# veeresht/CommPy

Measured on AMD Instinct MI355X. Metric: decoded info-bits/s at fixed Eb/N0 (Viterbi K=7 r=1/2, 1024b); BER match, higher is better.
Workload: dtype f64

## Files before the change

### commpy_amd/csrc/viterbi_cw.hip

```cpp
#include "cpx_internal.h"
#include "cpx_math.h"
#include "viterbi_cw_asm.h"
#ifndef CPX_GEN_GB
#define CPX_GEN_GB 2
#endif

#include <atomic>
#include <cstdlib>
#include <cstring>
#include <mutex>
#include <type_traits>

using namespace cpx;

namespace {

template <int LGS, unsigned G0, unsigned G1>
struct SrCode {
    static constexpr int S = 1 << LGS;
    static constexpr int parity(unsigned v) { return __builtin_popcount(v) & 1; }
    static constexpr int code(int s, int j) {
        const unsigned p = (unsigned)(((s << 1) & (S - 1)) | j), b = (unsigned)(s >> (LGS - 1));
        const unsigned reg = (b << LGS) | p;
        return (parity(reg & G0) << 1) | parity(reg & G1);
// ... 54 lines not shown
        m0 = (double)(ri ^ 0ll);
        m1 = (double)(ri ^ 1ll);
    } else if (type == CPX_VIT_SOFT) {
        double nll0 = fast_log<false>(exp(r) + 1.0);
        m0 = nll0;
        m1 = nll0 - r;
    } else {
        double d0 = r - (-1.0), d1 = r - 1.0;
        m0 = d0 * d0;
        m1 = d1 * d1;
    }
}

__device__ __forceinline__ double clip500(double r) {
    double c;
    asm("v_max_f64 %0, %1, %2\n\tv_min_f64 %0, %0, %3" : "=&v"(c) : "v"(r), "s"(-500.0), "s"(500.0));
    return c;
}
__device__ __forceinline__ void soft_metrics_lean(double r, double &m0, double &m1) {
    const double nll0 = fast_log<false, false, true>(exp_pm500(r) + 1.0);
    m0 = nll0;
    m1 = nll0 - r;
}

template <int LGS>
__device__ __forceinline__ unsigned tb_hop(unsigned long long w, unsigned st) {
    const unsigned hi = (unsigned)((w << (st & ((1u << LGS) - 1u))) >> 32);
    return __builtin_amdgcn_alignbit(st, hi, 31);
}

struct NoHook {
    template <int P> __device__ __forceinline__ void at() const {}
};

template <int LGS, unsigned G0, unsigned G1, int TYPE, int R, bool LEAN = false, class Hook = NoHook>
__device__ __forceinline__ void cw_step(double (&pm)[1 << LGS], double r0, double r1, unsigned long long &word, int &best,
                                        const Hook &hook = Hook(), unsigned char *bml = nullptr, const unsigned *gidx = nullptr) {
    constexpr int type = TYPE;
    using C = SrCode<LGS, G0, G1>;
    constexpr bool GEN = G0 == 0 && G1 == 0;
    constexpr int S = 1 << LGS, H = S / 2;
    double m00, m01, m10, m11;
    if constexpr (LEAN && TYPE == CPX_VIT_SOFT) {
        r0 = clip500(r0);
        r1 = clip500(r1);
        soft_metrics_lean(r0, m00, m01);
        soft_metrics_lean(r1, m10, m11);
    } else {
        if (type == CPX_VIT_SOFT) {
            r0 = fmin(fmax(r0, -500.0), 500.0);
            r1 = fmin(fmax(r1, -500.0), 500.0);
        }
        bit_metrics_cw(type, r0, m00, m01);
        bit_metrics_cw(type, r1, m10, m11);
    }
    double bmv[4];
    if constexpr (LEAN) {
        bmv[0] = m00 + m10; bmv[1] = m00 + m11;
        bmv[2] = m01 + m10; bmv[3] = m01 + m11;
    } else {
        bmv[0] = (0.0 + m00) + m10; bmv[1] = (0.0 + m00) + m11;
        bmv[2] = (0.0 + m01) + m10; bmv[3] = (0.0 + m01) + m11;
    }
    unsigned da = 0, db = 0;
    hook.template at<0>();
    auto butterfly = [&](int j, double m_a0, double m_a1, double m_b0, double m_b1) {
        const int x = rotl<LGS>(2 * j, R), y = rotl<LGS>(2 * j + 1, R);
        const double a = pm[x], b = pm[y];
        const double a0 = a + m_a0, a1 = b + m_a1;
        const double b0 = a + m_b0, b1 = b + m_b1;
        if (TYPE == CPX_VIT_UNQUANTIZED) {
            pm[x] = acs_select(da, a0, a1);
            pm[y] = acs_select(db, b0, b1);
        } else {
            pm[x] = acs_min(da, a0, a1);
            pm[y] = acs_min(db, b0, b1);
        }
    };
    if constexpr (GEN) {
        typedef double cpx_d4 __attribute__((ext_vector_type(4)));
        const cpx_d4 tab = {bmv[0], bmv[1], bmv[2], bmv[3]}, rtab = {bmv[3], bmv[2], bmv[1], bmv[0]};
        asm volatile("s_set_gpr_idx_on 0, 1" ::: "memory", "m0");
        auto acs_pair = [&](int j, double a0, double a1, double b0, double b1) {
            const int x = rotl<LGS>(2 * j, R), y = rotl<LGS>(2 * j + 1, R);
            if (TYPE == CPX_VIT_UNQUANTIZED) {
                pm[x] = acs_select(da, a0, a1);
                pm[y] = acs_select(db, b0, b1);
            } else {
                pm[x] = acs_min(da, a0, a1);
                pm[y] = acs_min(db, b0, b1);
            }
        };
        if constexpr (H >= 4 && TYPE != CPX_VIT_UNQUANTIZED) {
#pragma unroll
            for (int j = 0; j < H; j += 2) {
                if (j == H / 2) hook.template at<1>();
                const int x0 = rotl<LGS>(2 * j, R), y0 = rotl<LGS>(2 * j + 1, R), x1 = rotl<LGS>(2 * j + 2, R), y1 = rotl<LGS>(2 * j + 3, R);
                const double a = pm[x0], b = pm[y0], c = pm[x1], d = pm[y1];
                double a0, a1, b0, b1, c0, c1, d0, d1;
                asm volatile("s_set_gpr_idx_idx %[i0]\n\t"
                             "v_add_f64 %[a0], v[248:249], %[a]\n\t"
                             "v_add_f64 %[b1], v[248:249], %[b]\n\t"
                             "v_add_f64 %[a1], v[240:241], %[b]\n\t"
                             "v_add_f64 %[b0], v[240:241], %[a]\n\t"
                             "s_set_gpr_idx_idx %[i1]\n\t"
                             "v_add_f64 %[c0], v[248:249], %[c]\n\t"
                             "v_add_f64 %[d1], v[248:249], %[d]\n\t"
                             "v_add_f64 %[c1], v[240:241], %[d]\n\t"
                             "v_add_f64 %[d0], v[240:241], %[c]\n\t"
                             "s_set_gpr_idx_idx 0\n\t"
                             "v_cmp_lt_f64 vcc, %[a1], %[a0]\n\tv_addc_co_u32 %[da], vcc, %[da], %[da], vcc\n\tv_min_f64 %[a0], %[a0], %[a1]\n\t"
                             "v_cmp_lt_f64 vcc, %[b1], %[b0]\n\tv_addc_co_u32 %[db], vcc, %[db], %[db], vcc\n\tv_min_f64 %[b0], %[b0], %[b1]\n\t"
                             "v_cmp_lt_f64 vcc, %[c1], %[c0]\n\tv_addc_co_u32 %[da], vcc, %[da], %[da], vcc\n\tv_min_f64 %[c0], %[c0], %[c1]\n\t"
                             "v_cmp_lt_f64 vcc, %[d1], %[d0]\n\tv_addc_co_u32 %[db], vcc, %[db], %[db], vcc\n\tv_min_f64 %[d0], %[d0], %[d1]"
                             : [a0] "=&v"(a0), [a1] "=&v"(a1), [b0] "=&v"(b0), [b1] "=&v"(b1), [c0] "=&v"(c0), [c1] "=&v"(c1),
                               [d0] "=&v"(d0), [d1] "=&v"(d1), [da] "+v"(da), [db] "+v"(db)
                             : [i0] "s"(gidx[j]), [i1] "s"(gidx[j + 1]), [a] "v"(a), [b] "v"(b), [c] "v"(c), [d] "v"(d),
                               "{v[248:255]}"(tab), "{v[240:247]}"(rtab)
                             : "vcc", "m0");
                pm[x0] = a0; pm[y0] = b0;
                pm[x1] = c0; pm[y1] = d0;
            }
        } else {
#pragma unroll
            for (int j = 0; j < H; j++) {
                if (j == H / 2) hook.template at<1>();
                const double a = pm[rotl<LGS>(2 * j, R)], b = pm[rotl<LGS>(2 * j + 1, R)];
                double a0, a1, b0, b1;
                asm volatile("s_set_gpr_idx_idx %[ic]\n\t"
                             "v_add_f64 %[a0], v[248:249], %[a]\n\t"
                             "v_add_f64 %[b1], v[248:249], %[b]\n\t"
                             "v_add_f64 %[a1], v[240:241], %[b]\n\t"
                             "v_add_f64 %[b0], v[240:241], %[a]\n\t"
                             "s_set_gpr_idx_idx 0"
                             : [a0] "=&v"(a0), [a1] "=&v"(a1), [b0] "=&v"(b0), [b1] "=&v"(b1)
                             : [ic] "s"(gidx[j]), [a] "v"(a), [b] "v"(b), "{v[248:255]}"(tab), "{v[240:247]}"(rtab)
                             : "m0");
                acs_pair(j, a0, a1, b0, b1);
            }
        }
        asm volatile("s_set_gpr_idx_off" ::: "memory", "m0");
    } else {
#pragma unroll
        for (int j = 0; j < H; j++) {
            if (j == H / 2) hook.template at<1>();
            butterfly(j, bmv[C::code(j, 0)], bmv[C::code(j, 1)], bmv[C::code(j + H, 0)], bmv[C::code(j + H, 1)]);
        }
    }
    hook.template at<2>();
    int bst = 0;
    constexpr bool ARGMIN32 = LEAN && S == 64 && TYPE == CPX_VIT_SOFT && !GEN;
    unsigned long long tie = ~0ull;
    if constexpr (ARGMIN32) {
        unsigned h0, h1, h2, h3;
#define CPX_H4(a) "v"(__double2hiint(pm[a])), "v"(__double2hiint(pm[(a) + 1])), "v"(__double2hiint(pm[(a) + 2])), "v"(__double2hiint(pm[(a) + 3]))
        asm(CPX_HMIN_BLOCK0 : "=&v"(h0), "=&v"(h1), "=&v"(h2), "=&v"(h3) : CPX_H4(0), CPX_H4(4), CPX_H4(8), CPX_H4(12), CPX_H4(16));
        asm(CPX_HMIN_BLOCK1 : "+v"(h0), "+v"(h1), "+v"(h2), "+v"(h3) : CPX_H4(20), CPX_H4(24), CPX_H4(28), CPX_H4(32), CPX_H4(36), CPX_H4(40));
        asm(CPX_HMIN_BLOCK2 : "+v"(h0), "+v"(h1), "+v"(h2), "+v"(h3) : CPX_H4(44), CPX_H4(48), CPX_H4(52), CPX_H4(56), CPX_H4(60));
#undef CPX_H4
        hook.template at<3>();
        unsigned ha, hb, tmp;
#define CPX_P1(a) "v"(__double2hiint(pm[rotl<LGS>((a), R + 1)])), "v"(__double2hiint(pm[rotl<LGS>((a) + 32, R + 1)]))
#define CPX_P4(a) CPX_P1(a), CPX_P1((a) + 1), CPX_P1((a) + 2), CPX_P1((a) + 3)
        asm(CPX_HIT_BLOCK0 : "=&v"(ha), "=&v"(hb) : "v"(h0), CPX_P4(0), CPX_P4(4), CPX_P4(8) : "vcc");
        asm(CPX_HIT_BLOCK1 : "+v"(ha), "+v"(hb) : "v"(h0), CPX_P4(12), CPX_P4(16), CPX_P4(20) : "vcc");
        asm(CPX_HIT_BLOCK2 : "+v"(ha), "+v"(hb), "=&v"(bst), "=&v"(tmp), "=&s"(tie) : "v"(h0), CPX_P4(24), CPX_P4(28) : "vcc");
#undef CPX_P4
#undef CPX_P1
    }
    if (__builtin_expect(tie != 0, !ARGMIN32)) {
        double m0 = pm[0], m1 = pm[1 % S], m2 = pm[2 % S], m3 = pm[3 % S];
        if constexpr (S == 64) {
#define CPX_V4(a) "v"(pm[a]), "v"(pm[(a) + 1]), "v"(pm[(a) + 2]), "v"(pm[(a) + 3])
            asm(CPX_MIN_BLOCK24 : "+v"(m0), "+v"(m1), "+v"(m2), "+v"(m3)
                : CPX_V4(4), CPX_V4(8), CPX_V4(12), CPX_V4(16), CPX_V4(20), CPX_V4(24));
            asm(CPX_MIN_BLOCK24 : "+v"(m0), "+v"(m1), "+v"(m2), "+v"(m3)
                : CPX_V4(28), CPX_V4(32), CPX_V4(36), CPX_V4(40), CPX_V4(44), CPX_V4(48));
            asm(CPX_MIN_BLOCK12 : "+v"(m0), "+v"(m1), "+v"(m2), "+v"(m3) : CPX_V4(52), CPX_V4(56), CPX_V4(60));
#undef CPX_V4
        } else {
#pragma unroll
            for (int s = 4; s < S; s += 4) {
                m0 = vmin(m0, pm[s]); m1 = vmin(m1, pm[s + 1]); m2 = vmin(m2, pm[s + 2]); m3 = vmin(m3, pm[s + 3]);
            }
        }
        const double mn = vmin(vmin(m0, m1), vmin(m2, m3));
        if constexpr (!ARGMIN32) hook.template at<3>();
        if constexpr (S == 64) {
            unsigned long long k0, k1, k2, k3;
#define CPX_S4(a) "v"(pm[rotl<LGS>((a), R + 1)]), "v"(pm[rotl<LGS>((a) - 1, R + 1)]), "v"(pm[rotl<LGS>((a) - 2, R + 1)]), "v"(pm[rotl<LGS>((a) - 3, R + 1)])
            asm(CPX_SCAN_BLOCK0 : "+v"(bst), "=&s"(k0), "=&s"(k1), "=&s"(k2), "=&s"(k3)
                : "v"(mn), CPX_S4(63), CPX_S4(59), CPX_S4(55), CPX_S4(51), CPX_S4(47), CPX_S4(43));
            asm(CPX_SCAN_BLOCK1 : "+v"(bst), "=&s"(k0), "=&s"(k1), "=&s"(k2), "=&s"(k3)
                : "v"(mn), CPX_S4(39), CPX_S4(35), CPX_S4(31), CPX_S4(27), CPX_S4(23), CPX_S4(19));
            asm(CPX_SCAN_BLOCK2 : "+v"(bst), "=&s"(k0), "=&s"(k1), "=&s"(k2), "=&s"(k3)
                : "v"(mn), CPX_S4(15), CPX_S4(11), CPX_S4(7), CPX_S4(3));
#undef CPX_S4
        } else if constexpr (S % 4 == 0) {
#pragma unroll
            for (int s = S - 4; s >= 0; s -= 4) {
                unsigned long long k0, k1, k2, k3;
                asm("v_cmp_eq_f64 %1, %5, %9\n\tv_cmp_eq_f64 %2, %6, %9\n\tv_cmp_eq_f64 %3, %7, %9\n\tv_cmp_eq_f64 %4, %8, %9\n\t"
                    "v_cndmask_b32 %0, %0, %10, %1\n\tv_cndmask_b32 %0, %0, %11, %2\n\tv_cndmask_b32 %0, %0, %12, %3\n\t"
                    "v_cndmask_b32 %0, %0, %13, %4"
                    : "+v"(bst), "=&s"(k0), "=&s"(k1), "=&s"(k2), "=&s"(k3)
                    : "v"(pm[rotl<LGS>(s + 3, R + 1)]), "v"(pm[rotl<LGS>(s + 2, R + 1)]), "v"(pm[rotl<LGS>(s + 1, R + 1)]),
                      "v"(pm[rotl<LGS>(s, R + 1)]), "v"(mn), "n"(s + 3), "n"(s + 2), "n"(s + 1), "n"(s));
            }
        } else {
#pragma unroll
            for (int s = S - 1; s >= 0; s--) bst = (pm[rotl<LGS>(s, R + 1)] == mn) ? s : bst;
        }
    }
    word = ((unsigned long long)da << (64 - H)) | ((unsigned long long)db << (64 - S));
    best = bst;
}

__device__ __forceinline__ float acs_min_f32(unsigned &acc, float x, float y) {
    float r;
    asm("v_cmp_lt_f32 vcc, %3, %2\n\tv_addc_co_u32 %1, vcc, %1, %1, vcc\n\tv_min_f32 %0, %2, %3"
        : "=&v"(r), "+v"(acc) : "v"(x), "v"(y) : "vcc");
    return r;
}
__device__ __forceinline__ float vmin3_f32(float a, float b, float c) {
    float r;
    asm("v_min3_f32 %0, %1, %2, %3" : "=v"(r) : "v"(a), "v"(b), "v"(c));
    return r;
}
__device__ __forceinline__ void bit_metrics_f32(int type, double r, float &m0, float &m1) {
    if (type == CPX_VIT_HARD) {
        const long long ri = (long long)r;
        m0 = (float)(ri ^ 0ll);
        m1 = (float)(ri ^ 1ll);
    } else if (type == CPX_VIT_SOFT) {
        m0 = 0.0f;
        m1 = -(float)r;
    } else {
        const float x = (float)r, d0 = x + 1.0f, d1 = x - 1.0f;
        m0 = d0 * d0;
        m1 = d1 * d1;
    }
}

template <int LGS, unsigned G0, unsigned G1, int TYPE, int R, bool LEAN = false, class Hook = NoHook>
__device__ __forceinline__ void cw_step(float (&pm)[1 << LGS], double r0, double r1, unsigned long long &word, int &best,
                                        const Hook &hook = Hook(), unsigned char * = nullptr, const unsigned * = nullptr) {
    using C = SrCode<LGS, G0, G1>;
    constexpr int S = 1 << LGS, H = S / 2;
    if (TYPE == CPX_VIT_SOFT) {
        r0 = fmin(fmax(r0, -500.0), 500.0);
        r1 = fmin(fmax(r1, -500.0), 500.0);
    }
    float m00, m01, m10, m11;
    bit_metrics_f32(TYPE, r0, m00, m01);
    bit_metrics_f32(TYPE, r1, m10, m11);
    float bmv[4];
    bmv[0] = (0.0f + m00) + m10; bmv[1] = (0.0f + m00) + m11;
    bmv[2] = (0.0f + m01) + m10; bmv[3] = (0.0f + m01) + m11;
    unsigned da = 0, db = 0;
    hook.template at<0>();
#pragma unroll
    for (int j = 0; j < H; j++) {
        if (j == H / 2) hook.template at<1>();
        const int x = rotl<LGS>(2 * j, R), y = rotl<LGS>(2 * j + 1, R);
        const float a = pm[x], b = pm[y];
        const float a0 = a + bmv[C::code(j, 0)], a1 = b + bmv[C::code(j, 1)];
        const float b0 = a + bmv[C::code(j + H, 0)], b1 = b + bmv[C::code(j + H, 1)];
        pm[x] = acs_min_f32(da, a0, a1);
        pm[y] = acs_min_f32(db, b0, b1);
    }
    hook.template at<2>();
    float mn;
    if constexpr (S >= 8 && S % 8 == 0) {
        float m0 = pm[0], m1 = pm[1], m2 = pm[2], m3 = pm[3];
#pragma unroll
        for (int s = 4; s + 8 <= S; s += 8) {
            m0 = vmin3_f32(m0, pm[s], pm[s + 1]); m1 = vmin3_f32(m1, pm[s + 2], pm[s + 3]);
            m2 = vmin3_f32(m2, pm[s + 4], pm[s + 5]); m3 = vmin3_f32(m3, pm[s + 6], pm[s + 7]);
        }
        m0 = vmin3_f32(m0, pm[S - 4], pm[S - 3]);
        m1 = vmin3_f32(m1, pm[S - 2], pm[S - 1]);
        mn = fminf(vmin3_f32(m0, m1, m2), m3);
    } else {
        mn = pm[0];
#pragma unroll
        for (int s = 1; s < S; s++) mn = fminf(mn, pm[s]);
    }
    hook.template at<3>();
    int bst = 0;
    if constexpr (S % 4 == 0) {
#pragma unroll
        for (int s = S - 4; s >= 0; s -= 4) {
            unsigned long long k0, k1, k2, k3;
            asm("v_cmp_eq_f32 %1, %5, %9\n\tv_cmp_eq_f32 %2, %6, %9\n\tv_cmp_eq_f32 %3, %7, %9\n\tv_cmp_eq_f32 %4, %8, %9\n\t"
                "v_cndmask_b32 %0, %0, %10, %1\n\tv_cndmask_b32 %0, %0, %11, %2\n\tv_cndmask_b32 %0, %0, %12, %3\n\t"
                "v_cndmask_b32 %0, %0, %13, %4"
                : "+v"(bst), "=&s"(k0), "=&s"(k1), "=&s"(k2), "=&s"(k3)
                : "v"(pm[rotl<LGS>(s + 3, R + 1)]), "v"(pm[rotl<LGS>(s + 2, R + 1)]), "v"(pm[rotl<LGS>(s + 1, R + 1)]),
                  "v"(pm[rotl<LGS>(s, R + 1)]), "v"(mn), "n"(s + 3), "n"(s + 2), "n"(s + 1), "n"(s));
        }
    } else {
#pragma unroll
        for (int s = S - 1; s >= 0; s--) bst = (pm[rotl<LGS>(s, R + 1)] == mn) ? s : bst;
    }
    word = ((unsigned long long)da << (64 - H)) | ((unsigned long long)db << (64 - S));
    best = bst;
}

constexpr int ACS_WAVES = 4;

template <int LGS, unsigned G0, unsigned G1, int TYPE>
__global__ __launch_bounds__(64 * ACS_WAVES) void viterbi_cw_acs_kernel(CwParams p) {
    constexpr int S = 1 << LGS;
    const int lane = threadIdx.x & 63;
    const int64_t grp = (int64_t)blockIdx.x * ACS_WAVES + (threadIdx.x >> 6);
    const int64_t cw = grp * 64 + lane;
    if (grp * 64 >= p.B) return;
    const bool valid = cw < p.B;
    const double *x = p.coded + (valid ? cw : 0) * p.len;
    unsigned long long *dec = p.dec + grp * p.Tp * 64 + lane;
    unsigned char *best = p.best + grp * p.Tp * 64 + lane;
// ... 620 lines not shown
```

### commpy_amd/csrc/viterbi_cw_asm.h

```cpp
#pragma once
#define CPX_MIN_BLOCK24 "v_min_f64 %0, %0, %4\n\tv_min_f64 %1, %1, %5\n\tv_min_f64 %2, %2, %6\n\tv_min_f64 %3, %3, %7\n\tv_min_f64 %0, %0, %8\n\tv_min_f64 %1, %1, %9\n\tv_min_f64 %2, %2, %10\n\tv_min_f64 %3, %3, %11\n\tv_min_f64 %0, %0, %12\n\tv_min_f64 %1, %1, %13\n\tv_min_f64 %2, %2, %14\n\tv_min_f64 %3, %3, %15\n\tv_min_f64 %0, %0, %16\n\tv_min_f64 %1, %1, %17\n\tv_min_f64 %2, %2, %18\n\tv_min_f64 %3, %3, %19\n\tv_min_f64 %0, %0, %20\n\tv_min_f64 %1, %1, %21\n\tv_min_f64 %2, %2, %22\n\tv_min_f64 %3, %3, %23\n\tv_min_f64 %0, %0, %24\n\tv_min_f64 %1, %1, %25\n\tv_min_f64 %2, %2, %26\n\tv_min_f64 %3, %3, %27"
#define CPX_MIN_BLOCK12 "v_min_f64 %0, %0, %4\n\tv_min_f64 %1, %1, %5\n\tv_min_f64 %2, %2, %6\n\tv_min_f64 %3, %3, %7\n\tv_min_f64 %0, %0, %8\n\tv_min_f64 %1, %1, %9\n\tv_min_f64 %2, %2, %10\n\tv_min_f64 %3, %3, %11\n\tv_min_f64 %0, %0, %12\n\tv_min_f64 %1, %1, %13\n\tv_min_f64 %2, %2, %14\n\tv_min_f64 %3, %3, %15"
#define CPX_SCAN_BLOCK0 "v_cmp_eq_f64 %1, %6, %5\n\tv_cmp_eq_f64 %2, %7, %5\n\tv_cmp_eq_f64 %3, %8, %5\n\tv_cmp_eq_f64 %4, %9, %5\n\tv_cndmask_b32 %0, %0, 63, %1\n\tv_cndmask_b32 %0, %0, 62, %2\n\tv_cndmask_b32 %0, %0, 61, %3\n\tv_cndmask_b32 %0, %0, 60, %4\n\tv_cmp_eq_f64 %1, %10, %5\n\tv_cmp_eq_f64 %2, %11, %5\n\tv_cmp_eq_f64 %3, %12, %5\n\tv_cmp_eq_f64 %4, %13, %5\n\tv_cndmask_b32 %0, %0, 59, %1\n\tv_cndmask_b32 %0, %0, 58, %2\n\tv_cndmask_b32 %0, %0, 57, %3\n\tv_cndmask_b32 %0, %0, 56, %4\n\tv_cmp_eq_f64 %1, %14, %5\n\tv_cmp_eq_f64 %2, %15, %5\n\tv_cmp_eq_f64 %3, %16, %5\n\tv_cmp_eq_f64 %4, %17, %5\n\tv_cndmask_b32 %0, %0, 55, %1\n\tv_cndmask_b32 %0, %0, 54, %2\n\tv_cndmask_b32 %0, %0, 53, %3\n\tv_cndmask_b32 %0, %0, 52, %4\n\tv_cmp_eq_f64 %1, %18, %5\n\tv_cmp_eq_f64 %2, %19, %5\n\tv_cmp_eq_f64 %3, %20, %5\n\tv_cmp_eq_f64 %4, %21, %5\n\tv_cndmask_b32 %0, %0, 51, %1\n\tv_cndmask_b32 %0, %0, 50, %2\n\tv_cndmask_b32 %0, %0, 49, %3\n\tv_cndmask_b32 %0, %0, 48, %4\n\tv_cmp_eq_f64 %1, %22, %5\n\tv_cmp_eq_f64 %2, %23, %5\n\tv_cmp_eq_f64 %3, %24, %5\n\tv_cmp_eq_f64 %4, %25, %5\n\tv_cndmask_b32 %0, %0, 47, %1\n\tv_cndmask_b32 %0, %0, 46, %2\n\tv_cndmask_b32 %0, %0, 45, %3\n\tv_cndmask_b32 %0, %0, 44, %4\n\tv_cmp_eq_f64 %1, %26, %5\n\tv_cmp_eq_f64 %2, %27, %5\n\tv_cmp_eq_f64 %3, %28, %5\n\tv_cmp_eq_f64 %4, %29, %5\n\tv_cndmask_b32 %0, %0, 43, %1\n\tv_cndmask_b32 %0, %0, 42, %2\n\tv_cndmask_b32 %0, %0, 41, %3\n\tv_cndmask_b32 %0, %0, 40, %4"
#define CPX_SCAN_BLOCK1 "v_cmp_eq_f64 %1, %6, %5\n\tv_cmp_eq_f64 %2, %7, %5\n\tv_cmp_eq_f64 %3, %8, %5\n\tv_cmp_eq_f64 %4, %9, %5\n\tv_cndmask_b32 %0, %0, 39, %1\n\tv_cndmask_b32 %0, %0, 38, %2\n\tv_cndmask_b32 %0, %0, 37, %3\n\tv_cndmask_b32 %0, %0, 36, %4\n\tv_cmp_eq_f64 %1, %10, %5\n\tv_cmp_eq_f64 %2, %11, %5\n\tv_cmp_eq_f64 %3, %12, %5\n\tv_cmp_eq_f64 %4, %13, %5\n\tv_cndmask_b32 %0, %0, 35, %1\n\tv_cndmask_b32 %0, %0, 34, %2\n\tv_cndmask_b32 %0, %0, 33, %3\n\tv_cndmask_b32 %0, %0, 32, %4\n\tv_cmp_eq_f64 %1, %14, %5\n\tv_cmp_eq_f64 %2, %15, %5\n\tv_cmp_eq_f64 %3, %16, %5\n\tv_cmp_eq_f64 %4, %17, %5\n\tv_cndmask_b32 %0, %0, 31, %1\n\tv_cndmask_b32 %0, %0, 30, %2\n\tv_cndmask_b32 %0, %0, 29, %3\n\tv_cndmask_b32 %0, %0, 28, %4\n\tv_cmp_eq_f64 %1, %18, %5\n\tv_cmp_eq_f64 %2, %19, %5\n\tv_cmp_eq_f64 %3, %20, %5\n\tv_cmp_eq_f64 %4, %21, %5\n\tv_cndmask_b32 %0, %0, 27, %1\n\tv_cndmask_b32 %0, %0, 26, %2\n\tv_cndmask_b32 %0, %0, 25, %3\n\tv_cndmask_b32 %0, %0, 24, %4\n\tv_cmp_eq_f64 %1, %22, %5\n\tv_cmp_eq_f64 %2, %23, %5\n\tv_cmp_eq_f64 %3, %24, %5\n\tv_cmp_eq_f64 %4, %25, %5\n\tv_cndmask_b32 %0, %0, 23, %1\n\tv_cndmask_b32 %0, %0, 22, %2\n\tv_cndmask_b32 %0, %0, 21, %3\n\tv_cndmask_b32 %0, %0, 20, %4\n\tv_cmp_eq_f64 %1, %26, %5\n\tv_cmp_eq_f64 %2, %27, %5\n\tv_cmp_eq_f64 %3, %28, %5\n\tv_cmp_eq_f64 %4, %29, %5\n\tv_cndmask_b32 %0, %0, 19, %1\n\tv_cndmask_b32 %0, %0, 18, %2\n\tv_cndmask_b32 %0, %0, 17, %3\n\tv_cndmask_b32 %0, %0, 16, %4"
#define CPX_SCAN_BLOCK2 "v_cmp_eq_f64 %1, %6, %5\n\tv_cmp_eq_f64 %2, %7, %5\n\tv_cmp_eq_f64 %3, %8, %5\n\tv_cmp_eq_f64 %4, %9, %5\n\tv_cndmask_b32 %0, %0, 15, %1\n\tv_cndmask_b32 %0, %0, 14, %2\n\tv_cndmask_b32 %0, %0, 13, %3\n\tv_cndmask_b32 %0, %0, 12, %4\n\tv_cmp_eq_f64 %1, %10, %5\n\tv_cmp_eq_f64 %2, %11, %5\n\tv_cmp_eq_f64 %3, %12, %5\n\tv_cmp_eq_f64 %4, %13, %5\n\tv_cndmask_b32 %0, %0, 11, %1\n\tv_cndmask_b32 %0, %0, 10, %2\n\tv_cndmask_b32 %0, %0, 9, %3\n\tv_cndmask_b32 %0, %0, 8, %4\n\tv_cmp_eq_f64 %1, %14, %5\n\tv_cmp_eq_f64 %2, %15, %5\n\tv_cmp_eq_f64 %3, %16, %5\n\tv_cmp_eq_f64 %4, %17, %5\n\tv_cndmask_b32 %0, %0, 7, %1\n\tv_cndmask_b32 %0, %0, 6, %2\n\tv_cndmask_b32 %0, %0, 5, %3\n\tv_cndmask_b32 %0, %0, 4, %4\n\tv_cmp_eq_f64 %1, %18, %5\n\tv_cmp_eq_f64 %2, %19, %5\n\tv_cmp_eq_f64 %3, %20, %5\n\tv_cmp_eq_f64 %4, %21, %5\n\tv_cndmask_b32 %0, %0, 3, %1\n\tv_cndmask_b32 %0, %0, 2, %2\n\tv_cndmask_b32 %0, %0, 1, %3\n\tv_cndmask_b32 %0, %0, 0, %4"
#define CPX_HMIN_BLOCK0 "v_min3_u32 %0, %4, %8, %12\n\tv_min3_u32 %1, %5, %9, %13\n\tv_min3_u32 %2, %6, %10, %14\n\tv_min3_u32 %3, %7, %11, %15\n\tv_min3_u32 %0, %0, %16, %20\n\tv_min3_u32 %1, %1, %17, %21\n\tv_min3_u32 %2, %2, %18, %22\n\tv_min3_u32 %3, %3, %19, %23"
#define CPX_HMIN_BLOCK1 "v_min3_u32 %0, %0, %4, %8\n\tv_min3_u32 %1, %1, %5, %9\n\tv_min3_u32 %2, %2, %6, %10\n\tv_min3_u32 %3, %3, %7, %11\n\tv_min3_u32 %0, %0, %12, %16\n\tv_min3_u32 %1, %1, %13, %17\n\tv_min3_u32 %2, %2, %14, %18\n\tv_min3_u32 %3, %3, %15, %19\n\tv_min3_u32 %0, %0, %20, %24\n\tv_min3_u32 %1, %1, %21, %25\n\tv_min3_u32 %2, %2, %22, %26\n\tv_min3_u32 %3, %3, %23, %27"
#define CPX_HMIN_BLOCK2 "v_min3_u32 %0, %0, %4, %8\n\tv_min3_u32 %1, %1, %5, %9\n\tv_min3_u32 %2, %2, %6, %10\n\tv_min3_u32 %3, %3, %7, %11\n\tv_min3_u32 %0, %0, %12, %16\n\tv_min3_u32 %1, %1, %13, %17\n\tv_min3_u32 %2, %2, %14, %18\n\tv_min3_u32 %3, %3, %15, %19\n\tv_min3_u32 %0, %0, %20, %21\n\tv_min3_u32 %1, %1, %22, %23\n\tv_min3_u32 %0, %0, %2, %3\n\tv_min_u32 %0, %0, %1"
#define CPX_HIT_BLOCK0 "v_cmp_eq_u32 vcc, %2, %3\n\tv_cndmask_b32 %0, 0, 1, vcc\n\tv_cmp_eq_u32 vcc, %2, %4\n\tv_cndmask_b32 %1, 0, 1, vcc\n\tv_cmp_eq_u32 vcc, %2, %5\n\tv_addc_co_u32 %0, vcc, %0, %0, vcc\n\tv_cmp_eq_u32 vcc, %2, %6\n\tv_addc_co_u32 %1, vcc, %1, %1, vcc\n\tv_cmp_eq_u32 vcc, %2, %7\n\tv_addc_co_u32 %0, vcc, %0, %0, vcc\n\tv_cmp_eq_u32 vcc, %2, %8\n\tv_addc_co_u32 %1, vcc, %1, %1, vcc\n\tv_cmp_eq_u32 vcc, %2, %9\n\tv_addc_co_u32 %0, vcc, %0, %0, vcc\n\tv_cmp_eq_u32 vcc, %2, %10\n\tv_addc_co_u32 %1, vcc, %1, %1, vcc\n\tv_cmp_eq_u32 vcc, %2, %11\n\tv_addc_co_u32 %0, vcc, %0, %0, vcc\n\tv_cmp_eq_u32 vcc, %2, %12\n\tv_addc_co_u32 %1, vcc, %1, %1, vcc\n\tv_cmp_eq_u32 vcc, %2, %13\n\tv_addc_co_u32 %0, vcc, %0, %0, vcc\n\tv_cmp_eq_u32 vcc, %2, %14\n\tv_addc_co_u32 %1, vcc, %1, %1, vcc\n\tv_cmp_eq_u32 vcc, %2, %15\n\tv_addc_co_u32 %0, vcc, %0, %0, vcc\n\tv_cmp_eq_u32 vcc, %2, %16\n\tv_addc_co_u32 %1, vcc, %1, %1, vcc\n\tv_cmp_eq_u32 vcc, %2, %17\n\tv_addc_co_u32 %0, vcc, %0, %0, vcc\n\tv_cmp_eq_u32 vcc, %2, %18\n\tv_addc_co_u32 %1, vcc, %1, %1, vcc\n\tv_cmp_eq_u32 vcc, %2, %19\n\tv_addc_co_u32 %0, vcc, %0, %0, vcc\n\tv_cmp_eq_u32 vcc, %2, %20\n\tv_addc_co_u32 %1, vcc, %1, %1, vcc\n\tv_cmp_eq_u32 vcc, %2, %21\n\tv_addc_co_u32 %0, vcc, %0, %0, vcc\n\tv_cmp_eq_u32 vcc, %2, %22\n\tv_addc_co_u32 %1, vcc, %1, %1, vcc\n\tv_cmp_eq_u32 vcc, %2, %23\n\tv_addc_co_u32 %0, vcc, %0, %0, vcc\n\tv_cmp_eq_u32 vcc, %2, %24\n\tv_addc_co_u32 %1, vcc, %1, %1, vcc\n\tv_cmp_eq_u32 vcc, %2, %25\n\tv_addc_co_u32 %0, vcc, %0, %0, vcc\n\tv_cmp_eq_u32 vcc, %2, %26\n\tv_addc_co_u32 %1, vcc, %1, %1, vcc"
#define CPX_HIT_BLOCK1 "v_cmp_eq_u32 vcc, %2, %3\n\tv_addc_co_u32 %0, vcc, %0, %0, vcc\n\tv_cmp_eq_u32 vcc, %2, %4\n\tv_addc_co_u32 %1, vcc, %1, %1, vcc\n\tv_cmp_eq_u32 vcc, %2, %5\n\tv_addc_co_u32 %0, vcc, %0, %0, vcc\n\tv_cmp_eq_u32 vcc, %2, %6\n\tv_addc_co_u32 %1, vcc, %1, %1, vcc\n\tv_cmp_eq_u32 vcc, %2, %7\n\tv_addc_co_u32 %0, vcc, %0, %0, vcc\n\tv_cmp_eq_u32 vcc, %2, %8\n\tv_addc_co_u32 %1, vcc, %1, %1, vcc\n\tv_cmp_eq_u32 vcc, %2, %9\n\tv_addc_co_u32 %0, vcc, %0, %0, vcc\n\tv_cmp_eq_u32 vcc, %2, %10\n\tv_addc_co_u32 %1, vcc, %1, %1, vcc\n\tv_cmp_eq_u32 vcc, %2, %11\n\tv_addc_co_u32 %0, vcc, %0, %0, vcc\n\tv_cmp_eq_u32 vcc, %2, %12\n\tv_addc_co_u32 %1, vcc, %1, %1, vcc\n\tv_cmp_eq_u32 vcc, %2, %13\n\tv_addc_co_u32 %0, vcc, %0, %0, vcc\n\tv_cmp_eq_u32 vcc, %2, %14\n\tv_addc_co_u32 %1, vcc, %1, %1, vcc\n\tv_cmp_eq_u32 vcc, %2, %15\n\tv_addc_co_u32 %0, vcc, %0, %0, vcc\n\tv_cmp_eq_u32 vcc, %2, %16\n\tv_addc_co_u32 %1, vcc, %1, %1, vcc\n\tv_cmp_eq_u32 vcc, %2, %17\n\tv_addc_co_u32 %0, vcc, %0, %0, vcc\n\tv_cmp_eq_u32 vcc, %2, %18\n\tv_addc_co_u32 %1, vcc, %1, %1, vcc\n\tv_cmp_eq_u32 vcc, %2, %19\n\tv_addc_co_u32 %0, vcc, %0, %0, vcc\n\tv_cmp_eq_u32 vcc, %2, %20\n\tv_addc_co_u32 %1, vcc, %1, %1, vcc\n\tv_cmp_eq_u32 vcc, %2, %21\n\tv_addc_co_u32 %0, vcc, %0, %0, vcc\n\tv_cmp_eq_u32 vcc, %2, %22\n\tv_addc_co_u32 %1, vcc, %1, %1, vcc\n\tv_cmp_eq_u32 vcc, %2, %23\n\tv_addc_co_u32 %0, vcc, %0, %0, vcc\n\tv_cmp_eq_u32 vcc, %2, %24\n\tv_addc_co_u32 %1, vcc, %1, %1, vcc\n\tv_cmp_eq_u32 vcc, %2, %25\n\tv_addc_co_u32 %0, vcc, %0, %0, vcc\n\tv_cmp_eq_u32 vcc, %2, %26\n\tv_addc_co_u32 %1, vcc, %1, %1, vcc"
#define CPX_HIT_BLOCK2 "v_cmp_eq_u32 vcc, %5, %6\n\tv_addc_co_u32 %0, vcc, %0, %0, vcc\n\tv_cmp_eq_u32 vcc, %5, %7\n\tv_addc_co_u32 %1, vcc, %1, %1, vcc\n\tv_cmp_eq_u32 vcc, %5, %8\n\tv_addc_co_u32 %0, vcc, %0, %0, vcc\n\tv_cmp_eq_u32 vcc, %5, %9\n\tv_addc_co_u32 %1, vcc, %1, %1, vcc\n\tv_cmp_eq_u32 vcc, %5, %10\n\tv_addc_co_u32 %0, vcc, %0, %0, vcc\n\tv_cmp_eq_u32 vcc, %5, %11\n\tv_addc_co_u32 %1, vcc, %1, %1, vcc\n\tv_cmp_eq_u32 vcc, %5, %12\n\tv_addc_co_u32 %0, vcc, %0, %0, vcc\n\tv_cmp_eq_u32 vcc, %5, %13\n\tv_addc_co_u32 %1, vcc, %1, %1, vcc\n\tv_cmp_eq_u32 vcc, %5, %14\n\tv_addc_co_u32 %0, vcc, %0, %0, vcc\n\tv_cmp_eq_u32 vcc, %5, %15\n\tv_addc_co_u32 %1, vcc, %1, %1, vcc\n\tv_cmp_eq_u32 vcc, %5, %16\n\tv_addc_co_u32 %0, vcc, %0, %0, vcc\n\tv_cmp_eq_u32 vcc, %5, %17\n\tv_addc_co_u32 %1, vcc, %1, %1, vcc\n\tv_cmp_eq_u32 vcc, %5, %18\n\tv_addc_co_u32 %0, vcc, %0, %0, vcc\n\tv_cmp_eq_u32 vcc, %5, %19\n\tv_addc_co_u32 %1, vcc, %1, %1, vcc\n\tv_cmp_eq_u32 vcc, %5, %20\n\tv_addc_co_u32 %0, vcc, %0, %0, vcc\n\tv_cmp_eq_u32 vcc, %5, %21\n\tv_addc_co_u32 %1, vcc, %1, %1, vcc\n\tv_ffbh_u32 %2, %0\n\tv_ffbh_u32 %3, %1\n\tv_bcnt_u32_b32 %0, %0, 0\n\tv_add_u32 %3, 32, %3\n\tv_bcnt_u32_b32 %0, %1, %0\n\tv_min_u32 %2, %2, %3\n\tv_cmp_lt_u32 %4, 1, %0"
```

Baseline: 48.22 billion.

## Replace linear argmin hit-scan with 8x8 row/column min decomposition

The soft-decision K=7 argmin over 64 path metrics now treats the states as an 8x8 grid. It computes column minima and row minima of the high words, then builds two 8-bit hit masks and recovers the index from the first set bit of each. This replaces the 64 compare/add-with-carry scan that built 64-bit hit masks. The tie check changes to requiring exactly one matching row and one matching column. Rows and columns are both recomputed from the same inputs, so the VALU count may not fall much, and the tie-detection semantics are subtle.

```diff
diff --git a/commpy_amd/csrc/viterbi_cw.hip b/commpy_amd/csrc/viterbi_cw.hip
--- a/commpy_amd/csrc/viterbi_cw.hip
+++ b/commpy_amd/csrc/viterbi_cw.hip
@@ -230,21 +230,22 @@
     constexpr bool ARGMIN32 = LEAN && S == 64 && TYPE == CPX_VIT_SOFT && !GEN;
     unsigned long long tie = ~0ull;
     if constexpr (ARGMIN32) {
-        unsigned h0, h1, h2, h3;
-#define CPX_H4(a) "v"(__double2hiint(pm[a])), "v"(__double2hiint(pm[(a) + 1])), "v"(__double2hiint(pm[(a) + 2])), "v"(__double2hiint(pm[(a) + 3]))
-        asm(CPX_HMIN_BLOCK0 : "=&v"(h0), "=&v"(h1), "=&v"(h2), "=&v"(h3) : CPX_H4(0), CPX_H4(4), CPX_H4(8), CPX_H4(12), CPX_H4(16));
-        asm(CPX_HMIN_BLOCK1 : "+v"(h0), "+v"(h1), "+v"(h2), "+v"(h3) : CPX_H4(20), CPX_H4(24), CPX_H4(28), CPX_H4(32), CPX_H4(36), CPX_H4(40));
-        asm(CPX_HMIN_BLOCK2 : "+v"(h0), "+v"(h1), "+v"(h2), "+v"(h3) : CPX_H4(44), CPX_H4(48), CPX_H4(52), CPX_H4(56), CPX_H4(60));
-#undef CPX_H4
+#define CPX_HI(s) "v"(__double2hiint(pm[rotl<LGS>((s), R + 1)]))
+#define CPX_COL(i) CPX_HI(i), CPX_HI((i) + 8), CPX_HI((i) + 16), CPX_HI((i) + 24), CPX_HI((i) + 32), CPX_HI((i) + 40), CPX_HI((i) + 48), CPX_HI((i) + 56)
+#define CPX_ROW(j) CPX_HI(8 * (j)), CPX_HI(8 * (j) + 1), CPX_HI(8 * (j) + 2), CPX_HI(8 * (j) + 3), CPX_HI(8 * (j) + 4), CPX_HI(8 * (j) + 5), CPX_HI(8 * (j) + 6), CPX_HI(8 * (j) + 7)
+        unsigned q0, q1, q2, q3, q4, q5, q6, q7, m, w;
+        asm(CPX_COL_BLOCK3 : "=&v"(q0), "=&v"(q1), "=&v"(q2) : CPX_COL(0), CPX_COL(1), CPX_COL(2));
+        asm(CPX_COL_BLOCK3 : "=&v"(q3), "=&v"(q4), "=&v"(q5) : CPX_COL(3), CPX_COL(4), CPX_COL(5));
+        asm(CPX_COL_BLOCK_LAST : "=&v"(q6), "=&v"(q7), "=&v"(m), "=&v"(w) : "v"(q0), "v"(q1), "v"(q2), "v"(q3), "v"(q4), "v"(q5), CPX_COL(6), CPX_COL(7)
+            : "vcc");
         hook.template at<3>();
-        unsigned ha, hb, tmp;
-#define CPX_P1(a) "v"(__double2hiint(pm[rotl<LGS>((a), R + 1)])), "v"(__double2hiint(pm[rotl<LGS>((a) + 32, R + 1)]))
-#define CPX_P4(a) CPX_P1(a), CPX_P1((a) + 1), CPX_P1((a) + 2), CPX_P1((a) + 3)
-        asm(CPX_HIT_BLOCK0 : "=&v"(ha), "=&v"(hb) : "v"(h0), CPX_P4(0), CPX_P4(4), CPX_P4(8) : "vcc");
-        asm(CPX_HIT_BLOCK1 : "+v"(ha), "+v"(hb) : "v"(h0), CPX_P4(12), CPX_P4(16), CPX_P4(20) : "vcc");
-        asm(CPX_HIT_BLOCK2 : "+v"(ha), "+v"(hb), "=&v"(bst), "=&v"(tmp), "=&s"(tie) : "v"(h0), CPX_P4(24), CPX_P4(28) : "vcc");
-#undef CPX_P4
-#undef CPX_P1
+        unsigned r0_, r1_, r2_;
+        asm(CPX_ROW_BLOCK3 : "+v"(w), "=&v"(r0_), "=&v"(r1_), "=&v"(r2_) : "v"(m), CPX_ROW(7), CPX_ROW(6), CPX_ROW(5) : "vcc");
+        asm(CPX_ROW_BLOCK3 : "+v"(w), "=&v"(r0_), "=&v"(r1_), "=&v"(r2_) : "v"(m), CPX_ROW(4), CPX_ROW(3), CPX_ROW(2) : "vcc");
+        asm(CPX_ROW_BLOCK_LAST : "+v"(w), "=&v"(r0_), "=&v"(r1_), "=&v"(bst), "=&s"(tie) : "v"(m), CPX_ROW(1), CPX_ROW(0) : "vcc");
+#undef CPX_ROW
+#undef CPX_COL
+#undef CPX_HI
     }
     if (__builtin_expect(tie != 0, !ARGMIN32)) {
         double m0 = pm[0], m1 = pm[1 % S], m2 = pm[2 % S], m3 = pm[3 % S];
diff --git a/commpy_amd/csrc/viterbi_cw_asm.h b/commpy_amd/csrc/viterbi_cw_asm.h
--- a/commpy_amd/csrc/viterbi_cw_asm.h
+++ b/commpy_amd/csrc/viterbi_cw_asm.h
@@ -4,9 +4,7 @@
 #define CPX_SCAN_BLOCK0 "v_cmp_eq_f64 %1, %6, %5\n\tv_cmp_eq_f64 %2, %7, %5\n\tv_cmp_eq_f64 %3, %8, %5\n\tv_cmp_eq_f64 %4, %9, %5\n\tv_cndmask_b32 %0, %0, 63, %1\n\tv_cndmask_b32 %0, %0, 62, %2\n\tv_cndmask_b32 %0, %0, 61, %3\n\tv_cndmask_b32 %0, %0, 60, %4\n\tv_cmp_eq_f64 %1, %10, %5\n\tv_cmp_eq_f64 %2, %11, %5\n\tv_cmp_eq_f64 %3, %12, %5\n\tv_cmp_eq_f64 %4, %13, %5\n\tv_cndmask_b32 %0, %0, 59, %1\n\tv_cndmask_b32 %0, %0, 58, %2\n\tv_cndmask_b32 %0, %0, 57, %3\n\tv_cndmask_b32 %0, %0, 56, %4\n\tv_cmp_eq_f64 %1, %14, %5\n\tv_cmp_eq_f64 %2, %15, %5\n\tv_cmp_eq_f64 %3, %16, %5\n\tv_cmp_eq_f64 %4, %17, %5\n\tv_cndmask_b32 %0, %0, 55, %1\n\tv_cndmask_b32 %0, %0, 54, %2\n\tv_cndmask_b32 %0, %0, 53, %3\n\tv_cndmask_b32 %0, %0, 52, %4\n\tv_cmp_eq_f64 %1, %18, %5\n\tv_cmp_eq_f64 %2, %19, %5\n\tv_cmp_eq_f64 %3, %20, %5\n\tv_cmp_eq_f64 %4, %21, %5\n\tv_cndmask_b32 %0, %0, 51, %1\n\tv_cndmask_b32 %0, %0, 50, %2\n\tv_cndmask_b32 %0, %0, 49, %3\n\tv_cndmask_b32 %0, %0, 48, %4\n\tv_cmp_eq_f64 %1, %22, %5\n\tv_cmp_eq_f64 %2, %23, %5\n\tv_cmp_eq_f64 %3, %24, %5\n\tv_cmp_eq_f64 %4, %25, %5\n\tv_cndmask_b32 %0, %0, 47, %1\n\tv_cndmask_b32 %0, %0, 46, %2\n\tv_cndmask_b32 %0, %0, 45, %3\n\tv_cndmask_b32 %0, %0, 44, %4\n\tv_cmp_eq_f64 %1, %26, %5\n\tv_cmp_eq_f64 %2, %27, %5\n\tv_cmp_eq_f64 %3, %28, %5\n\tv_cmp_eq_f64 %4, %29, %5\n\tv_cndmask_b32 %0, %0, 43, %1\n\tv_cndmask_b32 %0, %0, 42, %2\n\tv_cndmask_b32 %0, %0, 41, %3\n\tv_cndmask_b32 %0, %0, 40, %4"
 #define CPX_SCAN_BLOCK1 "v_cmp_eq_f64 %1, %6, %5\n\tv_cmp_eq_f64 %2, %7, %5\n\tv_cmp_eq_f64 %3, %8, %5\n\tv_cmp_eq_f64 %4, %9, %5\n\tv_cndmask_b32 %0, %0, 39, %1\n\tv_cndmask_b32 %0, %0, 38, %2\n\tv_cndmask_b32 %0, %0, 37, %3\n\tv_cndmask_b32 %0, %0, 36, %4\n\tv_cmp_eq_f64 %1, %10, %5\n\tv_cmp_eq_f64 %2, %11, %5\n\tv_cmp_eq_f64 %3, %12, %5\n\tv_cmp_eq_f64 %4, %13, %5\n\tv_cndmask_b32 %0, %0, 35, %1\n\tv_cndmask_b32 %0, %0, 34, %2\n\tv_cndmask_b32 %0, %0, 33, %3\n\tv_cndmask_b32 %0, %0, 32, %4\n\tv_cmp_eq_f64 %1, %14, %5\n\tv_cmp_eq_f64 %2, %15, %5\n\tv_cmp_eq_f64 %3, %16, %5\n\tv_cmp_eq_f64 %4, %17, %5\n\tv_cndmask_b32 %0, %0, 31, %1\n\tv_cndmask_b32 %0, %0, 30, %2\n\tv_cndmask_b32 %0, %0, 29, %3\n\tv_cndmask_b32 %0, %0, 28, %4\n\tv_cmp_eq_f64 %1, %18, %5\n\tv_cmp_eq_f64 %2, %19, %5\n\tv_cmp_eq_f64 %3, %20, %5\n\tv_cmp_eq_f64 %4, %21, %5\n\tv_cndmask_b32 %0, %0, 27, %1\n\tv_cndmask_b32 %0, %0, 26, %2\n\tv_cndmask_b32 %0, %0, 25, %3\n\tv_cndmask_b32 %0, %0, 24, %4\n\tv_cmp_eq_f64 %1, %22, %5\n\tv_cmp_eq_f64 %2, %23, %5\n\tv_cmp_eq_f64 %3, %24, %5\n\tv_cmp_eq_f64 %4, %25, %5\n\tv_cndmask_b32 %0, %0, 23, %1\n\tv_cndmask_b32 %0, %0, 22, %2\n\tv_cndmask_b32 %0, %0, 21, %3\n\tv_cndmask_b32 %0, %0, 20, %4\n\tv_cmp_eq_f64 %1, %26, %5\n\tv_cmp_eq_f64 %2, %27, %5\n\tv_cmp_eq_f64 %3, %28, %5\n\tv_cmp_eq_f64 %4, %29, %5\n\tv_cndmask_b32 %0, %0, 19, %1\n\tv_cndmask_b32 %0, %0, 18, %2\n\tv_cndmask_b32 %0, %0, 17, %3\n\tv_cndmask_b32 %0, %0, 16, %4"
 #define CPX_SCAN_BLOCK2 "v_cmp_eq_f64 %1, %6, %5\n\tv_cmp_eq_f64 %2, %7, %5\n\tv_cmp_eq_f64 %3, %8, %5\n\tv_cmp_eq_f64 %4, %9, %5\n\tv_cndmask_b32 %0, %0, 15, %1\n\tv_cndmask_b32 %0, %0, 14, %2\n\tv_cndmask_b32 %0, %0, 13, %3\n\tv_cndmask_b32 %0, %0, 12, %4\n\tv_cmp_eq_f64 %1, %10, %5\n\tv_cmp_eq_f64 %2, %11, %5\n\tv_cmp_eq_f64 %3, %12, %5\n\tv_cmp_eq_f64 %4, %13, %5\n\tv_cndmask_b32 %0, %0, 11, %1\n\tv_cndmask_b32 %0, %0, 10, %2\n\tv_cndmask_b32 %0, %0, 9, %3\n\tv_cndmask_b32 %0, %0, 8, %4\n\tv_cmp_eq_f64 %1, %14, %5\n\tv_cmp_eq_f64 %2, %15, %5\n\tv_cmp_eq_f64 %3, %16, %5\n\tv_cmp_eq_f64 %4, %17, %5\n\tv_cndmask_b32 %0, %0, 7, %1\n\tv_cndmask_b32 %0, %0, 6, %2\n\tv_cndmask_b32 %0, %0, 5, %3\n\tv_cndmask_b32 %0, %0, 4, %4\n\tv_cmp_eq_f64 %1, %18, %5\n\tv_cmp_eq_f64 %2, %19, %5\n\tv_cmp_eq_f64 %3, %20, %5\n\tv_cmp_eq_f64 %4, %21, %5\n\tv_cndmask_b32 %0, %0, 3, %1\n\tv_cndmask_b32 %0, %0, 2, %2\n\tv_cndmask_b32 %0, %0, 1, %3\n\tv_cndmask_b32 %0, %0, 0, %4"
-#define CPX_HMIN_BLOCK0 "v_min3_u32 %0, %4, %8, %12\n\tv_min3_u32 %1, %5, %9, %13\n\tv_min3_u32 %2, %6, %10, %14\n\tv_min3_u32 %3, %7, %11, %15\n\tv_min3_u32 %0, %0, %16, %20\n\tv_min3_u32 %1, %1, %17, %21\n\tv_min3_u32 %2, %2, %18, %22\n\tv_min3_u32 %3, %3, %19, %23"
-#define CPX_HMIN_BLOCK1 "v_min3_u32 %0, %0, %4, %8\n\tv_min3_u32 %1, %1, %5, %9\n\tv_min3_u32 %2, %2, %6, %10\n\tv_min3_u32 %3, %3, %7, %11\n\tv_min3_u32 %0, %0, %12, %16\n\tv_min3_u32 %1, %1, %13, %17\n\tv_min3_u32 %2, %2, %14, %18\n\tv_min3_u32 %3, %3, %15, %19\n\tv_min3_u32 %0, %0, %20, %24\n\tv_min3_u32 %1, %1, %21, %25\n\tv_min3_u32 %2, %2, %22, %26\n\tv_min3_u32 %3, %3, %23, %27"
-#define CPX_HMIN_BLOCK2 "v_min3_u32 %0, %0, %4, %8\n\tv_min3_u32 %1, %1, %5, %9\n\tv_min3_u32 %2, %2, %6, %10\n\tv_min3_u32 %3, %3, %7, %11\n\tv_min3_u32 %0, %0, %12, %16\n\tv_min3_u32 %1, %1, %13, %17\n\tv_min3_u32 %2, %2, %14, %18\n\tv_min3_u32 %3, %3, %15, %19\n\tv_min3_u32 %0, %0, %20, %21\n\tv_min3_u32 %1, %1, %22, %23\n\tv_min3_u32 %0, %0, %2, %3\n\tv_min_u32 %0, %0, %1"
-#define CPX_HIT_BLOCK0 "v_cmp_eq_u32 vcc, %2, %3\n\tv_cndmask_b32 %0, 0, 1, vcc\n\tv_cmp_eq_u32 vcc, %2, %4\n\tv_cndmask_b32 %1, 0, 1, vcc\n\tv_cmp_eq_u32 vcc, %2, %5\n\tv_addc_co_u32 %0, vcc, %0, %0, vcc\n\tv_cmp_eq_u32 vcc, %2, %6\n\tv_addc_co_u32 %1, vcc, %1, %1, vcc\n\tv_cmp_eq_u32 vcc, %2, %7\n\tv_addc_co_u32 %0, vcc, %0, %0, vcc\n\tv_cmp_eq_u32 vcc, %2, %8\n\tv_addc_co_u32 %1, vcc, %1, %1, vcc\n\tv_cmp_eq_u32 vcc, %2, %9\n\tv_addc_co_u32 %0, vcc, %0, %0, vcc\n\tv_cmp_eq_u32 vcc, %2, %10\n\tv_addc_co_u32 %1, vcc, %1, %1, vcc\n\tv_cmp_eq_u32 vcc, %2, %11\n\tv_addc_co_u32 %0, vcc, %0, %0, vcc\n\tv_cmp_eq_u32 vcc, %2, %12\n\tv_addc_co_u32 %1, vcc, %1, %1, vcc\n\tv_cmp_eq_u32 vcc, %2, %13\n\tv_addc_co_u32 %0, vcc, %0, %0, vcc\n\tv_cmp_eq_u32 vcc, %2, %14\n\tv_addc_co_u32 %1, vcc, %1, %1, vcc\n\tv_cmp_eq_u32 vcc, %2, %15\n\tv_addc_co_u32 %0, vcc, %0, %0, vcc\n\tv_cmp_eq_u32 vcc, %2, %16\n\tv_addc_co_u32 %1, vcc, %1, %1, vcc\n\tv_cmp_eq_u32 vcc, %2, %17\n\tv_addc_co_u32 %0, vcc, %0, %0, vcc\n\tv_cmp_eq_u32 vcc, %2, %18\n\tv_addc_co_u32 %1, vcc, %1, %1, vcc\n\tv_cmp_eq_u32 vcc, %2, %19\n\tv_addc_co_u32 %0, vcc, %0, %0, vcc\n\tv_cmp_eq_u32 vcc, %2, %20\n\tv_addc_co_u32 %1, vcc, %1, %1, vcc\n\tv_cmp_eq_u32 vcc, %2, %21\n\tv_addc_co_u32 %0, vcc, %0, %0, vcc\n\tv_cmp_eq_u32 vcc, %2, %22\n\tv_addc_co_u32 %1, vcc, %1, %1, vcc\n\tv_cmp_eq_u32 vcc, %2, %23\n\tv_addc_co_u32 %0, vcc, %0, %0, vcc\n\tv_cmp_eq_u32 vcc, %2, %24\n\tv_addc_co_u32 %1, vcc, %1, %1, vcc\n\tv_cmp_eq_u32 vcc, %2, %25\n\tv_addc_co_u32 %0, vcc, %0, %0, vcc\n\tv_cmp_eq_u32 vcc, %2, %26\n\tv_addc_co_u32 %1, vcc, %1, %1, vcc"
-#define CPX_HIT_BLOCK1 "v_cmp_eq_u32 vcc, %2, %3\n\tv_addc_co_u32 %0, vcc, %0, %0, vcc\n\tv_cmp_eq_u32 vcc, %2, %4\n\tv_addc_co_u32 %1, vcc, %1, %1, vcc\n\tv_cmp_eq_u32 vcc, %2, %5\n\tv_addc_co_u32 %0, vcc, %0, %0, vcc\n\tv_cmp_eq_u32 vcc, %2, %6\n\tv_addc_co_u32 %1, vcc, %1, %1, vcc\n\tv_cmp_eq_u32 vcc, %2, %7\n\tv_addc_co_u32 %0, vcc, %0, %0, vcc\n\tv_cmp_eq_u32 vcc, %2, %8\n\tv_addc_co_u32 %1, vcc, %1, %1, vcc\n\tv_cmp_eq_u32 vcc, %2, %9\n\tv_addc_co_u32 %0, vcc, %0, %0, vcc\n\tv_cmp_eq_u32 vcc, %2, %10\n\tv_addc_co_u32 %1, vcc, %1, %1, vcc\n\tv_cmp_eq_u32 vcc, %2, %11\n\tv_addc_co_u32 %0, vcc, %0, %0, vcc\n\tv_cmp_eq_u32 vcc, %2, %12\n\tv_addc_co_u32 %1, vcc, %1, %1, vcc\n\tv_cmp_eq_u32 vcc, %2, %13\n\tv_addc_co_u32 %0, vcc, %0, %0, vcc\n\tv_cmp_eq_u32 vcc, %2, %14\n\tv_addc_co_u32 %1, vcc, %1, %1, vcc\n\tv_cmp_eq_u32 vcc, %2, %15\n\tv_addc_co_u32 %0, vcc, %0, %0, vcc\n\tv_cmp_eq_u32 vcc, %2, %16\n\tv_addc_co_u32 %1, vcc, %1, %1, vcc\n\tv_cmp_eq_u32 vcc, %2, %17\n\tv_addc_co_u32 %0, vcc, %0, %0, vcc\n\tv_cmp_eq_u32 vcc, %2, %18\n\tv_addc_co_u32 %1, vcc, %1, %1, vcc\n\tv_cmp_eq_u32 vcc, %2, %19\n\tv_addc_co_u32 %0, vcc, %0, %0, vcc\n\tv_cmp_eq_u32 vcc, %2, %20\n\tv_addc_co_u32 %1, vcc, %1, %1, vcc\n\tv_cmp_eq_u32 vcc, %2, %21\n\tv_addc_co_u32 %0, vcc, %0, %0, vcc\n\tv_cmp_eq_u32 vcc, %2, %22\n\tv_addc_co_u32 %1, vcc, %1, %1, vcc\n\tv_cmp_eq_u32 vcc, %2, %23\n\tv_addc_co_u32 %0, vcc, %0, %0, vcc\n\tv_cmp_eq_u32 vcc, %2, %24\n\tv_addc_co_u32 %1, vcc, %1, %1, vcc\n\tv_cmp_eq_u32 vcc, %2, %25\n\tv_addc_co_u32 %0, vcc, %0, %0, vcc\n\tv_cmp_eq_u32 vcc, %2, %26\n\tv_addc_co_u32 %1, vcc, %1, %1, vcc"
-#define CPX_HIT_BLOCK2 "v_cmp_eq_u32 vcc, %5, %6\n\tv_addc_co_u32 %0, vcc, %0, %0, vcc\n\tv_cmp_eq_u32 vcc, %5, %7\n\tv_addc_co_u32 %1, vcc, %1, %1, vcc\n\tv_cmp_eq_u32 vcc, %5, %8\n\tv_addc_co_u32 %0, vcc, %0, %0, vcc\n\tv_cmp_eq_u32 vcc, %5, %9\n\tv_addc_co_u32 %1, vcc, %1, %1, vcc\n\tv_cmp_eq_u32 vcc, %5, %10\n\tv_addc_co_u32 %0, vcc, %0, %0, vcc\n\tv_cmp_eq_u32 vcc, %5, %11\n\tv_addc_co_u32 %1, vcc, %1, %1, vcc\n\tv_cmp_eq_u32 vcc, %5, %12\n\tv_addc_co_u32 %0, vcc, %0, %0, vcc\n\tv_cmp_eq_u32 vcc, %5, %13\n\tv_addc_co_u32 %1, vcc, %1, %1, vcc\n\tv_cmp_eq_u32 vcc, %5, %14\n\tv_addc_co_u32 %0, vcc, %0, %0, vcc\n\tv_cmp_eq_u32 vcc, %5, %15\n\tv_addc_co_u32 %1, vcc, %1, %1, vcc\n\tv_cmp_eq_u32 vcc, %5, %16\n\tv_addc_co_u32 %0, vcc, %0, %0, vcc\n\tv_cmp_eq_u32 vcc, %5, %17\n\tv_addc_co_u32 %1, vcc, %1, %1, vcc\n\tv_cmp_eq_u32 vcc, %5, %18\n\tv_addc_co_u32 %0, vcc, %0, %0, vcc\n\tv_cmp_eq_u32 vcc, %5, %19\n\tv_addc_co_u32 %1, vcc, %1, %1, vcc\n\tv_cmp_eq_u32 vcc, %5, %20\n\tv_addc_co_u32 %0, vcc, %0, %0, vcc\n\tv_cmp_eq_u32 vcc, %5, %21\n\tv_addc_co_u32 %1, vcc, %1, %1, vcc\n\tv_ffbh_u32 %2, %0\n\tv_ffbh_u32 %3, %1\n\tv_bcnt_u32_b32 %0, %0, 0\n\tv_add_u32 %3, 32, %3\n\tv_bcnt_u32_b32 %0, %1, %0\n\tv_min_u32 %2, %2, %3\n\tv_cmp_lt_u32 %4, 1, %0"
+#define CPX_COL_BLOCK3 "v_min3_u32 %0, %3, %4, %5\n\tv_min3_u32 %1, %11, %12, %13\n\tv_min3_u32 %2, %19, %20, %21\n\tv_min3_u32 %0, %0, %6, %7\n\tv_min3_u32 %1, %1, %14, %15\n\tv_min3_u32 %2, %2, %22, %23\n\tv_min3_u32 %0, %0, %8, %9\n\tv_min3_u32 %1, %1, %16, %17\n\tv_min3_u32 %2, %2, %24, %25\n\tv_min_u32 %0, %0, %10\n\tv_min_u32 %1, %1, %18\n\tv_min_u32 %2, %2, %26"
+#define CPX_COL_BLOCK_LAST "v_min3_u32 %0, %10, %11, %12\n\tv_min3_u32 %1, %18, %19, %20\n\tv_min3_u32 %2, %4, %5, %6\n\tv_min3_u32 %0, %0, %13, %14\n\tv_min3_u32 %1, %1, %21, %22\n\tv_min3_u32 %3, %7, %8, %9\n\tv_min3_u32 %0, %0, %15, %16\n\tv_min3_u32 %1, %1, %23, %24\n\tv_min_u32 %0, %0, %17\n\tv_min_u32 %1, %1, %25\n\tv_min3_u32 %2, %2, %3, %0\n\tv_min_u32 %2, %2, %1\n\tv_cmp_eq_u32 vcc, %2, %1\n\tv_cndmask_b32 %3, 0, 1, vcc\n\tv_cmp_eq_u32 vcc, %2, %0\n\tv_addc_co_u32 %3, vcc, %3, %3, vcc\n\tv_cmp_eq_u32 vcc, %2, %9\n\tv_addc_co_u32 %3, vcc, %3, %3, vcc\n\tv_cmp_eq_u32 vcc, %2, %8\n\tv_addc_co_u32 %3, vcc, %3, %3, vcc\n\tv_cmp_eq_u32 vcc, %2, %7\n\tv_addc_co_u32 %3, vcc, %3, %3, vcc\n\tv_cmp_eq_u32 vcc, %2, %6\n\tv_addc_co_u32 %3, vcc, %3, %3, vcc\n\tv_cmp_eq_u32 vcc, %2, %5\n\tv_addc_co_u32 %3, vcc, %3, %3, vcc\n\tv_cmp_eq_u32 vcc, %2, %4\n\tv_addc_co_u32 %3, vcc, %3, %3, vcc"
+#define CPX_ROW_BLOCK3 "v_min3_u32 %1, %5, %6, %7\n\tv_min3_u32 %2, %13, %14, %15\n\tv_min3_u32 %3, %21, %22, %23\n\tv_min3_u32 %1, %1, %8, %9\n\tv_min3_u32 %2, %2, %16, %17\n\tv_min3_u32 %3, %3, %24, %25\n\tv_min3_u32 %1, %1, %10, %11\n\tv_min3_u32 %2, %2, %18, %19\n\tv_min3_u32 %3, %3, %26, %27\n\tv_min_u32 %1, %1, %12\n\tv_min_u32 %2, %2, %20\n\tv_min_u32 %3, %3, %28\n\tv_cmp_eq_u32 vcc, %4, %1\n\tv_addc_co_u32 %0, vcc, %0, %0, vcc\n\tv_cmp_eq_u32 vcc, %4, %2\n\tv_addc_co_u32 %0, vcc, %0, %0, vcc\n\tv_cmp_eq_u32 vcc, %4, %3\n\tv_addc_co_u32 %0, vcc, %0, %0, vcc"
+#define CPX_ROW_BLOCK_LAST "v_min3_u32 %1, %6, %7, %8\n\tv_min3_u32 %2, %14, %15, %16\n\tv_min3_u32 %1, %1, %9, %10\n\tv_min3_u32 %2, %2, %17, %18\n\tv_min3_u32 %1, %1, %11, %12\n\tv_min3_u32 %2, %2, %19, %20\n\tv_min_u32 %1, %1, %13\n\tv_min_u32 %2, %2, %21\n\tv_cmp_eq_u32 vcc, %5, %1\n\tv_addc_co_u32 %0, vcc, %0, %0, vcc\n\tv_cmp_eq_u32 vcc, %5, %2\n\tv_addc_co_u32 %0, vcc, %0, %0, vcc\n\tv_ffbl_b32 %3, %0\n\tv_lshrrev_b32 %1, 8, %0\n\tv_bcnt_u32_b32 %2, %0, 0\n\tv_ffbl_b32 %1, %1\n\tv_cmp_ne_u32 %4, 2, %2\n\tv_lshl_or_b32 %3, %3, 3, %1"
```

Result: faster. 51.96 billion (median of 6 runs) (+7.8%).
